# LBruyne/Scalable-Collaborative-zkSNARK

Measured on AMD Instinct MI355X. Metric: G1 scalar-muls/sec (d_msm) + Fr field-ops/sec (d_sumcheck), 2^20 shares, 1/2/4/8 GPU, higher is better.
Workload: dtype u32

## Files before the change

scalable-collaborative-zksnark_amd/csrc/zk_api.cpp:

```cpp
#include <cstdarg>
#include <cstdio>
#include <cstdlib>
#include <cstring>
#include <mutex>
#include <string>
#include <vector>

#include "zk_ctx.hpp"

namespace zk {

struct TuneKey {
    const char* name;
    long Tuning::*field;
};
static const TuneKey kTuneKeys[] = {
    {"sc_pass_wg", &Tuning::sc_pass_wg}, {"sc_local_g", &Tuning::sc_local_g}, {"sc_local_threads", &Tuning::sc_local_threads}, {"sc_ts", &Tuning::sc_ts}, {"sc_xcd", &Tuning::sc_xcd},
    {"sc_kf", &Tuning::sc_kf}, {"sc_plain_flat", &Tuning::sc_plain_flat}, {"sc_kp", &Tuning::sc_kp}, {"sc_k0", &Tuning::sc_k0},
    {"sc_flat_wg", &Tuning::sc_flat_wg}, {"sc_plain_wg", &Tuning::sc_plain_wg}, {"sc_pre", &Tuning::sc_pre},
    {"sc_pinned_out", &Tuning::sc_pinned_out}, {"sc_t1_device", &Tuning::sc_t1_device}, {"sc_handover", &Tuning::sc_handover},
    {"gate_local_e", &Tuning::gate_local_e}, {"gate_pass_wg", &Tuning::gate_pass_wg},
    {"wiring_local_e", &Tuning::wiring_local_e}, {"wiring_pass_wg", &Tuning::wiring_pass_wg},
    {"multi_local_e", &Tuning::multi_local_e}, {"multi_pass_wg", &Tuning::multi_pass_wg},
    {"perm3_local_e", &Tuning::perm3_local_e}, {"gatew_local_e", &Tuning::gatew_local_e},
    {"lookup_local_e", &Tuning::lookup_local_e}, {"lookupsel_local_e", &Tuning::lookupsel_local_e},
    {"msm_table_dc", &Tuning::msm_table_dc}, {"msm_qstep", &Tuning::msm_qstep}, {"msm_tile", &Tuning::msm_tile}, {"msm_pair", &Tuning::msm_pair},
    {"msm_fixq", &Tuning::msm_fixq}, {"msm_quad", &Tuning::msm_quad}, {"msm_stage", &Tuning::msm_stage}, {"msm_split", &Tuning::msm_split},
    {"msm_np", &Tuning::msm_np}, {"msm_fused_min", &Tuning::msm_fused_min}, {"msm_l2_tiled", &Tuning::msm_l2_tiled}, {"msm_tab_spt", &Tuning::msm_tab_spt}, {"msm_idx_ahead", &Tuning::msm_idx_ahead}, {"msm_share_l1", &Tuning::msm_share_l1}, {"srs_table_batched", &Tuning::srs_table_batched}, {"msm_debug", &Tuning::msm_debug}, {"msm_serial", &Tuning::msm_serial}, {"msm_size_classes", &Tuning::msm_size_classes},
    {"g1_map_by_column", &Tuning::g1_map_by_column}, {"msm_share", &Tuning::msm_share}, {"srs_table_rec", &Tuning::srs_table_rec}, {"msm_size_class_min", &Tuning::msm_size_class_min}, {"msm_small_table_widths", &Tuning::msm_small_table_widths},
};
static Tuning g_tuning;
int tune_set(const char* key, long value) {
    if (!key) return ZK_ERR_INVALID;
    for (const TuneKey& k : kTuneKeys)
        if (!std::strcmp(k.name, key)) {
            tuning().*(k.field) = value;
            return ZK_OK;
        }
    return ZK_ERR_INVALID;
}
Tuning& tuning() {
    static std::once_flag once;
    std::call_once(once, [] {
        const char* e = std::getenv("ZKHIP_TUNE");
        if (!e) return;
        std::string s(e);
        size_t pos = 0;
        while (pos < s.size()) {
            size_t end = s.find(',', pos);
            if (end == std::string::npos) end = s.size();
            const std::string kv = s.substr(pos, end - pos);
            const size_t eq = kv.find('=');
            bool ok = false;
            if (eq != std::string::npos) {
                const std::string k = kv.substr(0, eq);
                for (const TuneKey& t : kTuneKeys)
                    if (k == t.name) {
                        g_tuning.*(t.field) = std::atol(kv.c_str() + eq + 1);
                        ok = true;
                    }
// ... 675 lines not shown
```

scalable-collaborative-zksnark_amd/csrc/zk_ctx.hpp:

```cpp
#pragma once
#include <hip/hip_runtime.h>
#include <stdint.h>
#include <mutex>
#include <string>
#include <unordered_map>
#include <vector>

#include "../../include/zkhip.h"
#include "../../include/zkhip_test.h"

struct zk_msm_job;

struct zk_srs {
    void* d_bases = nullptr;
    size_t n = 0;
    bool owned = true;
    bool g2 = false;
    void* d_table = nullptr;
    int table_c = 0;
    size_t table_stride = 0;
    size_t table_rec = 96;
};

struct zk_ctx {
// ... 65 lines not shown
    long sc_pass_wg = 0;
    long sc_local_g = 256;
    long sc_local_threads = 1024;
    long sc_ts = 0;
    long sc_xcd = 1;
    long sc_kf = 4;
    long sc_plain_flat = 1;
    long sc_kp = 2;
    long sc_k0 = 3;
    long sc_flat_wg = 64;
    long sc_plain_wg = 3;
    long sc_pre = 1;
    long sc_pinned_out = 1;
    long sc_handover = 1;
    long sc_t1_device = 0;
    long gate_local_e = 512;
    long gate_pass_wg = 0;
    long wiring_local_e = 512;
    long wiring_pass_wg = 0;
    long multi_local_e = 512;
    long multi_pass_wg = 0;
    long perm3_local_e = 256;
    long gatew_local_e = 256;
    long lookup_local_e = 512;
    long lookupsel_local_e = 512;
    long msm_table_dc = 0;
    long msm_qstep = 2;
    long msm_tile = 0;
    long msm_pair = 0;
    long msm_fixq = 65536;
    long msm_quad = 32768;
    long msm_stage = -1;
    long msm_split = 1;
    long msm_np = 0;
    long msm_fused_min = 0;
    long msm_share_l1 = 1;
    long msm_idx_ahead = 1;
    long msm_tab_spt = 0;
    long msm_l2_tiled = 0;
    long msm_debug = 0;
    long msm_serial = 0;
    long msm_size_classes = 1;
    long srs_table_batched = 1;
    long srs_table_rec = 0;
    long msm_size_class_min = 16;
    long msm_small_table_widths = 1;
    long msm_share = 100;
    long g1_map_by_column = 1;
};
Tuning& tuning();
int tune_set(const char* key, long value);

int fail(zk_ctx* ctx, int code, const char* fmt, ...);
int hip_fail(zk_ctx* ctx, hipError_t e, const char* what);
void* scratch(zk_ctx* ctx, int slot, size_t bytes);
void* pinned(zk_ctx* ctx, size_t bytes);
hipError_t device_alloc(zk_ctx* ctx, void** out, size_t bytes, bool pool_locked = false);
size_t pool_trim(zk_ctx* ctx);
int msm_lanes_reserve(zk_ctx* ctx, int lane, const uint64_t* caps10, uint64_t pinned_cap);

#define ZK_HIP(ctx, call)                                            \
    do {                                                             \
        hipError_t _e = (call);                                      \
        if (_e != hipSuccess) return zk::hip_fail(ctx, _e, #call);   \
    } while (0)

// ... 100 lines not shown
```

scalable-collaborative-zksnark_amd/csrc/zk_msm.hip:

```cpp
#include "curve30.cuh"
#include "curve30_g2.cuh"
#include "host_curve.hpp"
#include "zk_ctx.hpp"

#include <algorithm>
#include <chrono>
#include <cstdio>
#include <cstdlib>
#include <condition_variable>
#include <cstring>
#include <deque>
#include <functional>
#include <mutex>
#include <thread>
#include <vector>

namespace zk {

static constexpr int kBlk = 256;
static constexpr u32 kSkip = 0xffffffffu;


struct CvG1 {
    typedef Aff30 Aff;
// ... 858 lines not shown
    return 0;
}
static void tab_launch_hist(int c, dim3 grid, hipStream_t st, const ItemDesc* items, WinLayout L, u32 chunk_sc, u32 nchunks, u32 np, int low_bits, u32* hist) {
    switch (c) {
#define X(Cc) case Cc: hipLaunchKernelGGL(k_tab_hist<Cc>, grid, dim3(kSortThreads), 0, st, items, L, chunk_sc, nchunks, np, low_bits, hist); break;
        ZK_TAB_WIDTHS(X)
#undef X
        default: hipLaunchKernelGGL(k_tab_hist<0>, grid, dim3(kSortThreads), 0, st, items, L, chunk_sc, nchunks, np, low_bits, hist);
    }
}
template <int SPT, int C>
static void tab_launch_scatter_one(dim3 grid, size_t lds, hipStream_t st, const ItemDesc* items, u32 ns, WinLayout L, u32 nchunks, u32 np, int low_bits, const u32* hist,
                                   const u32* ptotal, const u32* base, int idx_bits, size_t row_len, u32* part_idx, unsigned short* part_low) {
    hipFuncSetAttribute((const void*)k_tab_scatter<SPT, C>, hipFuncAttributeMaxDynamicSharedMemorySize, 160 * 1024);
    hipLaunchKernelGGL((k_tab_scatter<SPT, C>), grid, dim3(kSortThreads), lds, st, items, ns, L, nchunks, np, low_bits, hist, ptotal, base, idx_bits, row_len, part_idx, part_low);
}
static void tab_launch_scatter(int c, int spt, dim3 grid, size_t lds, hipStream_t st, const ItemDesc* items, u32 ns, WinLayout L, u32 nchunks, u32 np, int low_bits,
                               const u32* hist, const u32* ptotal, const u32* base, int idx_bits, size_t row_len, u32* part_idx, unsigned short* part_low) {
#define ZK_ARGS grid, lds, st, items, ns, L, nchunks, np, low_bits, hist, ptotal, base, idx_bits, row_len, part_idx, part_low
    switch (c) {
#define X(Cc) case Cc: if (spt == 2) tab_launch_scatter_one<2, Cc>(ZK_ARGS); else tab_launch_scatter_one<1, Cc>(ZK_ARGS); break;
        ZK_TAB_WIDTHS(X)
#undef X
        default: if (spt == 2) tab_launch_scatter_one<2, 0>(ZK_ARGS); else tab_launch_scatter_one<1, 0>(ZK_ARGS);
    }
#undef ZK_ARGS
}

template <class Cv>
static __global__ void __launch_bounds__(kBlk) k_accum_tiles(const ItemDesc* __restrict__ items, int rows_per_item,
                                                    const u32* __restrict__ sorted, const uint2* __restrict__ oc_all,
                                                    const u32* __restrict__ tile_b, size_t ns, u32 nsi, int nsi_shift, size_t nb, u32 T,
                                                    size_t tiles_per_w, size_t total_tiles, void* __restrict__ buckets,
                                                    void* __restrict__ heads, void* __restrict__ tails, int idx_ahead) {
  for (size_t g = (size_t)blockIdx.x * kBlk + threadIdx.x; g < total_tiles; g += (size_t)gridDim.x * kBlk) {
    const size_t w = g / tiles_per_w, t = g % tiles_per_w;
    const ItemDesc it = items[w / rows_per_item];
    const void* __restrict__ bases = it.bases;
    auto pidx = [&](u32 v) -> size_t {
        v &= 0x7fffffffu;
        if (it.pstride == 0) return v;
        const u32 win = nsi_shift >= 0 ? (v >> nsi_shift) : v / nsi;
        return (size_t)win * it.pstride + (v - win * nsi);
    };
    const uint2* oc = oc_all + w * nb;
    const uint2 last = oc[nb - 1];
    const u32 nw = last.x + last.y;
    const u32 e0 = (u32)t * T;
    if (e0 >= nw) continue;
    const u32 e1 = (e0 + T < nw) ? e0 + T : nw;
    u32 b = tile_b[g];
    uint2 cur_b = oc[b];
    u32 bstart = cur_b.x, bend = cur_b.x + cur_b.y;
    u32 ps = e0;
    const u32* run = sorted + w * ns;
    typename Cv::Xyzz acc;
    Cv::set_inf(acc);
    u32 v = run[e0];
    u32 vn = (idx_ahead && e0 + 1 < e1) ? run[e0 + 1] : 0u;
    typename Cv::Aff p = Cv::aff_load_rec(bases, pidx(v), it.rec);
    for (u32 e = e0; e < e1; e++) {
        if (e == bend) {
            if (ps == bstart) Cv::store(buckets, w * nb + b, acc);
            else Cv::store(heads, g, acc);
            do {
                b++;
                cur_b = oc[b];
                bstart = cur_b.x;
                bend = cur_b.x + cur_b.y;
            } while (bend == bstart);
            ps = e;
            Cv::set_inf(acc);
        }
        const bool neg = (v >> 31) != 0;
        typename Cv::Aff cur = p;
        if (e + 1 < e1) {
            if (idx_ahead) {
                v = vn;
                if (e + 2 < e1) vn = run[e + 2];
            } else {
                v = run[e + 1];
            }
            p = Cv::aff_load_rec(bases, pidx(v), it.rec);
        }
        Cv::madd(acc, cur, neg);
    }
    if (ps == bstart && e1 == bend) Cv::store(buckets, w * nb + b, acc);
    else if (ps == e0) Cv::store(heads, g, acc);
    else Cv::store(tails, g, acc);
  }
}

struct NarrowRows {
    int rpi, w0, from;
    __host__ __device__ bool narrow(size_t row) const { return w0 + (int)(row % (size_t)rpi) >= from; }
};

static constexpr u32 kLongSpan = 24;
template <class Cv>
static __global__ void __launch_bounds__(kBlk) k_fixup(const uint2* __restrict__ oc, size_t nb, NarrowRows nr, u32 T,
                                              size_t tiles_per_w, size_t total, void* __restrict__ buckets,
                                              const void* __restrict__ heads, const void* __restrict__ tails,
                                              u32* __restrict__ long_count, u32* __restrict__ long_list) {
    const size_t g = (size_t)blockIdx.x * kBlk + threadIdx.x;
    if (g >= total) return;
    const size_t w = g / nb;
    if (nr.narrow(w) && (g % nb) >= nb / 2) return;
    const uint2 ocg = oc[g];
    const u32 s = ocg.x, c = ocg.y;
    if (c == 0) {
        typename Cv::Xyzz z;
        Cv::set_inf(z);
        Cv::store(buckets, g, z);
        return;
    }
    const u32 e = s + c;
    const u32 t0 = s / T, t1 = (e - 1) / T;
    if (t0 == t1) return;
    if (t1 - t0 > kLongSpan) {
        long_list[atomicAdd(long_count, 1u)] = (u32)g;
        return;
    }
    const size_t base = w * tiles_per_w;
    typename Cv::Xyzz acc = (s == t0 * T) ? Cv::load(heads, base + t0) : Cv::load(tails, base + t0);
    for (u32 t = t0 + 1; t <= t1; t++) acc = Cv::add(acc, Cv::load(heads, base + t));
    Cv::store(buckets, g, acc);
}

template <class Cv>
static __global__ void __launch_bounds__(kBlk) k_fixup_quad(const uint2* __restrict__ oc, size_t nb, NarrowRows nr, u32 T,
                                                   size_t tiles_per_w, size_t total, void* __restrict__ buckets,
                                                   const void* __restrict__ heads, const void* __restrict__ tails,
                                                   u32* __restrict__ long_count, u32* __restrict__ long_list) {
    const size_t tq = (size_t)blockIdx.x * kBlk + threadIdx.x;
    const size_t g = tq >> 2;
    const int role = (int)(tq & 3);
    if (g >= total) return;
    const size_t w = g / nb;
    if (nr.narrow(w) && (g % nb) >= nb / 2) return;
    const uint2 ocg = oc[g];
    const u32 s = ocg.x, c = ocg.y;
    if (c == 0) {
        Cv::quad_store_inf(buckets, g, role);
        return;
    }
    const u32 e = s + c;
    const u32 t0 = s / T, t1 = (e - 1) / T;
    if (t0 == t1) return;
    if (t1 - t0 > kLongSpan) {
        if (role == 0) long_list[atomicAdd(long_count, 1u)] = (u32)g;
        return;
    }
    const size_t base = w * tiles_per_w;
    typename Cv::Xyzz acc = (s == t0 * T) ? Cv::load(heads, base + t0) : Cv::load(tails, base + t0);
    for (u32 t = t0 + 1; t <= t1; t++) acc = Cv::acc_quad(acc, heads, base + t, role);
    Cv::quad_store(buckets, g, role, acc);
}

template <class Cv>
static __global__ void __launch_bounds__(kBlk) k_fixup_long(const uint2* __restrict__ oc, size_t nb, u32 T,
                                                   size_t tiles_per_w, void* __restrict__ buckets, const void* __restrict__ heads,
                                                   const void* __restrict__ tails, const u32* __restrict__ long_count,
                                                   const u32* __restrict__ long_list) {
    extern __shared__ uint4 red[];
    const u32 nlong = *long_count;
    for (u32 i = blockIdx.x; i < nlong; i += gridDim.x) {
        const size_t g = long_list[i];
        const size_t w = g / nb;
// ... 282 lines not shown
    std::memcpy(Y.data(), p + 6, 48);
    std::memcpy(ZZ.data(), p + 12, 48);
    std::memcpy(ZZZ.data(), p + 18, 48);
    if (zkhost::is_zero(ZZ)) return zkhost::jac_inf();
    return zkhost::xyzz_to_jac(zkhost::mul(X, zkhost::K378()), zkhost::mul(Y, zkhost::K378()), zkhost::mul(ZZ, zkhost::K378()),
                               zkhost::mul(ZZZ, zkhost::K378()));
}

template <class HF>
static void combine_windows(zkhost::JacT<HF>& acc, const uint64_t* h, const WinLayout& L, int w0, int wc, int c, int nout, bool pair) {
    typedef zkhost::JacT<HF> J;
    constexpr size_t fw = zkhost::fe_words<HF>();
    const size_t p_lo = (size_t)L.bit_offset(w0);
    const size_t p_hi = (w0 + wc >= L.W) ? (size_t)L.bit_offset(L.W - 1) + L.width(L.W - 1) + c + 2 : (size_t)L.bit_offset(w0 + wc);
    std::vector<J> pos(p_hi - p_lo, zkhost::jac_inf_t<HF>());
    for (int w = 0; w < wc; w++) {
        for (int j = 0; j < nout; j++) {
            const uint64_t* src = h + ((size_t)w * nout + j) * 3 * fw;
            J pt;
            zkhost::get_fe(pt.x, src);
            zkhost::get_fe(pt.y, src + fw);
            zkhost::get_fe(pt.z, src + 2 * fw);
            if (zkhost::is_zero(pt.z)) continue;
            const size_t p = (size_t)L.bit_offset(w0 + w) + (pair ? 2 * (size_t)j : (j == c - 1 ? 0 : (size_t)j)) - p_lo;
            pos[p] = zkhost::jac_add(pos[p], pt);
        }
    }
    for (size_t p = pos.size(); p-- > 0;) {
        acc = zkhost::jac_dbl(acc);
        if (!zkhost::is_zero(pos[p].z)) acc = zkhost::jac_add(acc, pos[p]);
    }
}

struct HostPool {
    std::vector<std::thread> th;
    std::mutex mu;
    std::condition_variable cv, cv_done;
    std::deque<std::function<void()>> q;
    size_t pending = 0;
    bool stop = false;
    explicit HostPool(unsigned n) {
        for (unsigned i = 0; i < n; i++)
            th.emplace_back([this] {
                for (;;) {
                    std::function<void()> job;
                    {
                        std::unique_lock<std::mutex> lk(mu);
                        cv.wait(lk, [this] { return stop || !q.empty(); });
                        if (q.empty()) return;
                        job = std::move(q.front());
                        q.pop_front();
                    }
                    job();
                    {
                        std::lock_guard<std::mutex> lk(mu);
                        if (--pending == 0) cv_done.notify_all();
                    }
                }
            });
    }
    void submit(std::function<void()> f) {
        {
            std::lock_guard<std::mutex> lk(mu);
            q.push_back(std::move(f));
            pending++;
        }
// ... 19 lines not shown
#ifndef ZK_MSM_TU_G2
void msm_host_pool_destroy(zk_ctx* ctx) {
    delete (HostPool*)ctx->host_pool;
    ctx->host_pool = nullptr;
}

#endif
struct MsmClass {
    bool shared = false;
    int rpi = 0;
    size_t row_len = 0;
    int copies = 2;
    int c = 0;
    int key_c = 0;
    int size_key = 0;
    int narrow_from = 0x7fffffff;
    int w0 = 0, wc = 0;
    int part = 0, nparts = 1;
    int npair = 0;
    bool pair = false;
    WinLayout L{};
    std::vector<size_t> idx;
    size_t ns = 0, nb = 0, rows = 0, total = 0, tiles_per_w = 0, total_tiles = 0, chunk_len = 0, cc_elems = 0;
    u32 T = 32, nchunks = 0, np = 1;
    int low_bits = 0;
    int idx_bits = 0;
    bool staged_scatter = false;
    bool fused_tab = false;
    bool tiled_l2 = false;
    u32 tab_spt = 2;
    int tab_c = 0;
    u32 l2_ub = 0;
    size_t pinned_off = 0;
    size_t off[10] = {0, 0, 0, 0, 0, 0, 0, 0, 0, 0};
};

static int quantised_window(int c) {
    const int step = std::max(1, (int)tuning().msm_qstep);
    return c <= 5 ? 5 : (c > 17 ? 19 : std::min(17, 5 + step * ((c - 5 + step - 1) / step)));
}

struct MsmRun {
    int lane = 0;
    bool own_mem = false;
    size_t count = 0;
    std::vector<MsmItem> items;
    std::vector<MsmClass> classes;
    std::vector<size_t> empty_items;
    void* buf[10] = {};
    char* hpin = nullptr;
    size_t pinned_bytes = 0;
    size_t accum_wg_cap = 0;
};

static void msm_release(zk_ctx* ctx, MsmRun& run) {
    if (!run.own_mem || run.lane <= 0) return;
    ctx->lanes[run.lane].busy = false;
    run.lane = -1;
}

static int msm_lane_prepare(zk_ctx* ctx, int lane) {
    zk_ctx::MsmLane& L = ctx->lanes[lane];
    if (lane == 0) L.main = ctx->stream;
    if (L.ready) return ZK_OK;
    ZK_HIP(ctx, hipStreamCreateWithFlags(&L.main, hipStreamNonBlocking));
    for (auto& s2 : L.aux) ZK_HIP(ctx, hipStreamCreateWithFlags(&s2, hipStreamNonBlocking));
// ... 187 lines not shown
            cl.np = (u32)std::min<size_t>(cl.nb, want);
        }
        cl.low_bits = 0;
        while (((size_t)cl.np << cl.low_bits) < cl.nb) cl.low_bits++;
        {
            int ib = 1;
            while (((size_t)1 << ib) < cl.row_len) ib++;
            cl.idx_bits = (ib + cl.low_bits <= 31) ? ib : 0;
        }
        cl.staged_scatter = stage_env >= 0 ? stage_env != 0 : cl.row_len >= ((size_t)1 << 20);
        if (cl.rows * (size_t)cl.np * (cl.row_len / kStageChunk + 1) > ((size_t)64 << 20)) cl.staged_scatter = false;
        cl.chunk_len = cl.staged_scatter ? kStageChunk : (std::max<size_t>(16384, (cl.row_len + 511) / 512) + 3) & ~(size_t)3;
        cl.nchunks = (u32)((cl.row_len + cl.chunk_len - 1) / cl.chunk_len);
        cl.fused_tab = cl.shared && cl.w0 == 0 && cl.wc == cl.L.W && cl.L.W <= kTabW && cl.np == kMaxParts && cl.row_len >= ((size_t)1 << (tn.msm_fused_min > 0 ? tn.msm_fused_min : 23)) &&
                       tn.msm_fused_min >= 0;
        if (cl.fused_tab) {
            cl.tab_spt = cl.L.W <= 16 ? 2 : 1;
            if (tn.msm_tab_spt == 1) cl.tab_spt = 1;
            cl.tab_c = tab_width_known(cl.key_c);
            if (cl.tab_c) {
                const WinLayout chk = msm_layout(cl.tab_c, kFullBits);
                if (chk.W != cl.L.W || chk.base != cl.L.base || chk.rem != cl.L.rem) cl.tab_c = 0;
            }
            const size_t chunk_sc = (size_t)cl.tab_spt * kSortThreads;
            const size_t nch = (cl.ns + chunk_sc - 1) / chunk_sc;
            if (cl.rows * (size_t)cl.np * nch > ((size_t)64 << 20)) cl.fused_tab = false;
            else cl.nchunks = (u32)nch;
        }
        cl.tiled_l2 = tn.msm_l2_tiled >= 0 && cl.row_len / cl.np >= (size_t)(tn.msm_l2_tiled > 0 ? tn.msm_l2_tiled : 8192) && (tn.msm_l2_tiled > 0 || cl.row_len >= ((size_t)1 << 23));
        cl.l2_ub = (u32)(cl.row_len / kL2Tile + cl.np);
        if (cl.tiled_l2 && cl.rows * (size_t)cl.l2_ub * ((size_t)1 << cl.low_bits) > ((size_t)64 << 20)) cl.tiled_l2 = false;
        cl.cc_elems = cl.rows * (size_t)cl.np * cl.nchunks + 2 * cl.rows * (size_t)cl.np + cl.rows;
        if (cl.tiled_l2) cl.cc_elems += cl.rows * (size_t)(cl.np + 1) + cl.rows * (size_t)cl.l2_ub * ((size_t)1 << cl.low_bits);
        const size_t total64 = (cl.total + 63) & ~(size_t)63, tiles64 = (cl.total_tiles + 63) & ~(size_t)63;
        const size_t want_b[10] = {cl.rows * cl.row_len * 4, cl.rows * cl.row_len * 4, 2 * cl.total * 4 + cl.total_tiles * 4, total64 * Cv::kXyzzBytes, total64 * Cv::kXyzzBytes,
                                   2 * tiles64 * Cv::kXyzzBytes, (cl.total_tiles / kLongSpan + 64 + 1) * 4, nitems * sizeof(ItemDesc),
                                   cl.cc_elems * 4, cl.rows * cl.row_len * 2};
        for (int i = 0; i < 10; i++) {
            const bool shared_scratch = share_l1 && (i == 1 || i == 9);
            cl.off[i] = shared_scratch ? 0 : need[i];
            if (shared_scratch) need[i] = std::max(need[i], (want_b[i] + 255) & ~(size_t)255);
            else need[i] += (want_b[i] + 255) & ~(size_t)255;
        }
        cl.pinned_off = pinned_bytes;
        pinned_bytes += ((cl.rows * (size_t)cl.npair * Cv::kJacBytes + 255) & ~(size_t)255) + ((nitems * sizeof(ItemDesc) + 255) & ~(size_t)255);
    }
    const bool dbg_classes = tn.msm_debug != 0;
    if (dbg_classes)
        for (auto& cl : classes) {
            size_t nmin = ~(size_t)0, nmax2 = 0, tot = 0;
            for (size_t k : cl.idx) nmin = std::min(nmin, items[k].n), nmax2 = std::max(nmax2, items[k].n), tot += items[k].n;
            fprintf(stderr, "zk-class key_c=%d c=%d W=%d items=%zu n=[%zu..%zu] sum=%zu ns=%zu rows=%zu nb=%zu buckets=%zu T=%u tiles=%zu np=%u\n", cl.key_c, cl.c, cl.wc,
                    cl.idx.size(), nmin, nmax2, tot, cl.ns, cl.rows, cl.nb, cl.total, cl.T, cl.total_tiles, cl.np);
        }
    static const int slot[10] = {0, 1, 2, 3, 4, 5, 6, 9, 8, 11};
    void** buf = run.buf;
    run.pinned_bytes = pinned_bytes;
    if (run.own_mem) {
        int pick = -1;
        size_t pick_cap = 0;
        bool pick_fits = false;
        for (int l = 1; l < zk_ctx::kLanes; l++) {
            const zk_ctx::MsmLane& cand = ctx->lanes[l];
            if (cand.busy) continue;
            size_t cap = 0;
            bool fits = cand.pinned_cap >= pinned_bytes;
            for (int i = 0; i < 10; i++) cap += cand.mem[i].cap, fits = fits && cand.mem[i].cap >= need[i];
            const bool better = pick < 0 || (fits && !pick_fits) || (fits == pick_fits && (fits ? cap < pick_cap : cap > pick_cap));
            if (better) pick = l, pick_cap = cap, pick_fits = fits;
        }
        if (pick < 0) return fail(ctx, ZK_ERR_INVALID, "too many asynchronous MSM jobs in flight (at most %d): wait for one first", zk_ctx::kLanes - 1);
        run.lane = pick;
        {
            const int rc = msm_lane_prepare(ctx, run.lane);
            if (rc) return rc;
        }
        zk_ctx::MsmLane& LL = ctx->lanes[run.lane];
        for (int i = 0; i < 10; i++) {
            zk_ctx::Arena& a = LL.mem[i];
            if (a.cap < need[i] || !a.p) {
                if (a.p) hipFree(a.p);
                a.p = nullptr, a.cap = 0;
                const size_t want = std::max<size_t>(need[i], 256);
                const hipError_t e = device_alloc(ctx, &a.p, want);
                if (e != hipSuccess) {
                    a.p = nullptr;
// ... 40 lines not shown
    const bool multi = classes.size() > 1 && !serial_env;
    if (multi) {
        hipEventRecord(L.ev_fork, L.main);
        for (int k = 0; k < zk_ctx::kAux; k++) hipStreamWaitEvent(L.aux[k], L.ev_fork, 0);
    }
#define ZK_HIP_INFLIGHT(ctx, call)                                   \
    do {                                                             \
        hipError_t _e = (call);                                      \
        if (_e != hipSuccess) {                                      \
            hipDeviceSynchronize();                                  \
            msm_release(ctx, run);                                   \
            return zk::hip_fail(ctx, _e, #call);                     \
        }                                                            \
    } while (0)
    size_t cls_i = 0;
    for (auto& cl : classes) {
        const size_t nitems = cl.idx.size(), ns = cl.ns, nb = cl.nb, total = cl.total;
        const bool t_first = timers && (cls_i == 0), t_last = timers && (cls_i + 1 == (size_t)classes[0].nparts);
        hipStream_t st = (!multi || cls_i == 0) ? L.main : L.aux[(cls_i - 1) % zk_ctx::kAux];
        u32* digits = (u32*)((char*)buf[0] + cl.off[0]);
        u32* sorted = digits;
        u32* part_idx = (u32*)((char*)buf[1] + cl.off[1]);
        unsigned short* part_low = (unsigned short*)((char*)buf[9] + cl.off[9]);
        uint2* oc = (uint2*)((char*)buf[2] + cl.off[2]);
        u32* tile_b = (u32*)(oc + total);
        void* bufA = (char*)buf[3] + cl.off[3];
        void* bufB = (char*)buf[4] + cl.off[4];
        void* heads = (char*)buf[5] + cl.off[5];
        void* tails = (char*)heads + ((cl.total_tiles + 63) & ~(size_t)63) * Cv::kXyzzBytes;
        u32* longs = (u32*)((char*)buf[6] + cl.off[6]);
        ItemDesc* d_items = (ItemDesc*)((char*)buf[7] + cl.off[7]);
        u32* cc = (u32*)((char*)buf[8] + cl.off[8]);
        uint64_t* h_pts = (uint64_t*)(hpin + cl.pinned_off);
        ItemDesc* h_items = (ItemDesc*)(hpin + cl.pinned_off + ((cl.rows * (size_t)cl.npair * Cv::kJacBytes + 255) & ~(size_t)255));
        for (size_t j = 0; j < nitems; j++) {
            const MsmItem& it = items[cl.idx[j]];
            h_items[j].scalars = it.d_scalars;
            h_items[j].rec = cl.shared ? (u32)it.srs->table_rec : (u32)Cv::kAffBytes;
            h_items[j].bases = (const char*)(cl.shared ? it.srs->d_table : it.srs->d_bases) + it.offset * (size_t)h_items[j].rec;
            h_items[j].n = (u32)it.n;
            h_items[j].pstride = cl.shared ? (u32)it.srs->table_stride : (Cv::kEndo ? (u32)it.srs->n : 0u);
        }
        if (t_first) hipEventRecord(ctx->ev[0], st);
        ZK_HIP_INFLIGHT(ctx, hipMemcpyAsync(d_items, h_items, nitems * sizeof(ItemDesc), hipMemcpyHostToDevice, st));
        ZK_HIP_INFLIGHT(ctx, hipMemsetAsync(longs, 0, 4, st));
        if (share_l1) {
            while (L.ev_sort.size() <= cls_i) {
                hipEvent_t e = nullptr;
                ZK_HIP_INFLIGHT(ctx, hipEventCreateWithFlags(&e, hipEventDisableTiming));
                L.ev_sort.push_back(e);
            }
            if (cls_i > 0) hipStreamWaitEvent(st, L.ev_sort[cls_i - 1], 0);
        }
        if (!cl.fused_tab)
            hipLaunchKernelGGL(k_digits, dim3((unsigned)((ns + kBlk - 1) / kBlk), (unsigned)nitems), dim3(kBlk), 0, st,
                               (const ItemDesc*)d_items, ns, cl.L, cl.w0, cl.wc, (cl.shared || !Cv::kEndo) ? 0 : 1, digits);
        {
            u32* hist = cc;
            u32* ptotal = hist + cl.rows * (size_t)cl.np * cl.nchunks;
            u32* pbase = ptotal + cl.rows * (size_t)cl.np;
            u32* rowtot = pbase + cl.rows * (size_t)cl.np;
            const dim3 g_chunks((unsigned)(cl.nchunks * cl.rows)), g_parts((unsigned)(cl.np * cl.rows));
            const RowReal rr{(const ItemDesc*)d_items, (u32)cl.rpi, (u32)ns};
            if (cl.fused_tab)
                tab_launch_hist(cl.tab_c, g_chunks, st, (const ItemDesc*)d_items, cl.L, cl.tab_spt * (u32)kSortThreads, cl.nchunks, cl.np, cl.low_bits, hist);
            else
                hipLaunchKernelGGL(k_part_hist, g_chunks, dim3(kSortThreads), 0, st, (const u32*)digits, cl.row_len, cl.chunk_len, cl.nchunks, cl.np,
// ... 5 lines not shown
                tab_launch_scatter(cl.tab_c, (int)cl.tab_spt, dim3((unsigned)(8 * ((cl.nchunks + 7) / 8) * cl.rows)), lds, st, (const ItemDesc*)d_items, (u32)ns, cl.L, cl.nchunks, cl.np, cl.low_bits, (const u32*)hist,
                                   (const u32*)ptotal, (const u32*)pbase, cl.idx_bits, cl.row_len, part_idx, part_low);
            } else if (cl.staged_scatter) {
                const size_t lds = (3 * (size_t)kMaxParts + kSortThreads + 2 * (size_t)kStageChunk) * 4;
                hipFuncSetAttribute((const void*)k_part_scatter_staged, hipFuncAttributeMaxDynamicSharedMemorySize, 160 * 1024);
                hipLaunchKernelGGL(k_part_scatter_staged, g_chunks, dim3(kSortThreads), lds, st, (const u32*)digits, cl.row_len, cl.chunk_len,
                                   cl.nchunks, cl.np, cl.low_bits, (const u32*)hist, (const u32*)pbase, cl.idx_bits, part_idx, part_low, rr);
            } else {
                hipLaunchKernelGGL(k_part_scatter, g_chunks, dim3(kSortThreads), 0, st, (const u32*)digits, cl.row_len, cl.chunk_len, cl.nchunks,
                                   cl.np, cl.low_bits, (const u32*)hist, (const u32*)pbase, cl.idx_bits, part_idx, part_low, rr);
            }
            if (cl.tiled_l2) {
                u32* tstart = rowtot + cl.rows;
                u32* h2 = tstart + cl.rows * (size_t)(cl.np + 1);
                const u32 ub = cl.l2_ub;
                const dim3 g_tiles((unsigned)(ub * cl.rows));
                const size_t lds = (2 * ((size_t)1 << cl.low_bits) + 1 + 160 + kL2Tile) * 4;
                hipLaunchKernelGGL(k_l2_tiles, dim3((unsigned)cl.rows), dim3(kScanThreads), 0, st, (const u32*)pbase, (const u32*)rowtot, cl.np, tstart);
                hipLaunchKernelGGL(k_l2_hist, g_tiles, dim3(kSortThreads), 0, st, (const u32*)part_idx, (const unsigned short*)part_low, cl.row_len, cl.np, cl.low_bits, cl.idx_bits,
                                   (const u32*)pbase, (const u32*)rowtot, (const u32*)tstart, ub, h2);
                hipLaunchKernelGGL(k_l2_scan, g_parts, dim3(kSortThreads), 0, st, cl.np, cl.low_bits, nb, (const u32*)pbase, (const u32*)tstart, ub, h2, oc, cl.T, cl.tiles_per_w, tile_b);
                hipFuncSetAttribute((const void*)k_l2_scatter, hipFuncAttributeMaxDynamicSharedMemorySize, 160 * 1024);
                hipLaunchKernelGGL(k_l2_scatter, dim3((unsigned)(8 * ((ub + 7) / 8) * cl.rows)), dim3(kSortThreads), lds, st, (const u32*)part_idx, (const unsigned short*)part_low, cl.row_len, cl.np, cl.low_bits,
                                   cl.idx_bits, nb, (const u32*)pbase, (const u32*)rowtot, (const u32*)tstart, ub, (const u32*)h2, (const uint2*)oc, sorted);
            } else
            hipLaunchKernelGGL(k_part_sort, g_parts, dim3(cl.row_len / cl.np >= 4096 ? kSortThreads : 256), 0, st, (const u32*)part_idx, (const unsigned short*)part_low, cl.row_len,
                               cl.np, cl.low_bits, cl.idx_bits, nb, (const u32*)pbase, (const u32*)rowtot, oc, cl.T, cl.tiles_per_w, tile_b, sorted);
        }
        if (share_l1) hipEventRecord(L.ev_sort[cls_i], st);
        if (t_first) hipEventRecord(ctx->ev[1], st);
        if (cl.part > 0) hipStreamWaitEvent(st, L.ev_part[(cl.part - 1) % zk_ctx::kParts], 0);
        const size_t accum_wgs_full = (cl.total_tiles + kBlk - 1) / kBlk;
        const size_t accum_wgs = run.accum_wg_cap ? std::min<size_t>(accum_wgs_full, run.accum_wg_cap) : accum_wgs_full;
        hipLaunchKernelGGL((k_accum_tiles<Cv>), dim3((unsigned)accum_wgs), dim3(kBlk), 0, st,
                           (const ItemDesc*)d_items, cl.rpi, (const u32*)sorted, (const uint2*)oc, (const u32*)tile_b, cl.row_len,
                           (u32)ns, ((ns & (ns - 1)) == 0) ? (int)__builtin_ctzll(ns) : -1, nb, cl.T, cl.tiles_per_w, cl.total_tiles, bufA, heads, tails, (int)tn.msm_idx_ahead);
        if (cl.nparts > 1 && cl.part + 1 < cl.nparts) hipEventRecord(L.ev_part[cl.part % zk_ctx::kParts], st);
        if (t_last) hipEventRecord(ctx->ev[4], st);
        const NarrowRows nrw{cl.rpi, cl.w0, cl.narrow_from};
        if (Cv::kQuad && total <= fixq_max)
            hipLaunchKernelGGL((k_fixup_quad<Cv>), dim3((unsigned)((4 * total + kBlk - 1) / kBlk)), dim3(kBlk), 0, st, (const uint2*)oc,
                               nb, nrw, cl.T, cl.tiles_per_w, total, bufA, (const void*)heads, (const void*)tails, longs,
                               longs + 1);
        else
            hipLaunchKernelGGL((k_fixup<Cv>), dim3((unsigned)((total + kBlk - 1) / kBlk)), dim3(kBlk), 0, st, (const uint2*)oc,
                               nb, nrw, cl.T, cl.tiles_per_w, total, bufA, (const void*)heads, (const void*)tails, longs,
                               longs + 1);
        hipLaunchKernelGGL((k_fixup_long<Cv>), dim3(512), dim3(Cv::kXyzzBytes == 192 ? kBlk : kBlk / 2), (size_t)48 * 1024, st, (const uint2*)oc, nb, cl.T,
                           cl.tiles_per_w, bufA, (const void*)heads, (const void*)tails, (const u32*)longs, (const u32*)(longs + 1));
        if (t_last) hipEventRecord(ctx->ev[2], st);
        void* in = bufA;
        void* out = bufB;
        int rows = 1;
        size_t len = nb;
        while (len > 1) {
            size_t threads = cl.rows * (size_t)(rows + 1) * (len >> 1);
            if (Cv::kQuad && threads <= quad_max)
                hipLaunchKernelGGL((k_halve_quad<Cv>), dim3((unsigned)((4 * threads + kBlk - 1) / kBlk)), dim3(kBlk), 0, st, (const void*)in, out,
                                   (int)cl.rows, rows, len, nrw);
            else
                hipLaunchKernelGGL((k_halve<Cv>), dim3((unsigned)((threads + kBlk - 1) / kBlk)), dim3(kBlk), 0, st, (const void*)in, out,
                                   (int)cl.rows, rows, len, nrw);
            std::swap(in, out);
            rows++;
            len >>= 1;
        }
        {
            const size_t threads = cl.rows * (size_t)cl.npair;
            hipLaunchKernelGGL((k_finish<Cv>), dim3((unsigned)((threads + 63) / 64)), dim3(64), 0, st, (const void*)in, out, cl.rows, cl.c, cl.npair, cl.pair ? 1 : 0);
        }
        ZK_HIP_INFLIGHT(ctx, hipGetLastError());
        ZK_HIP_INFLIGHT(ctx, hipMemcpyAsync(h_pts, out, cl.rows * (size_t)cl.npair * Cv::kJacBytes, hipMemcpyDeviceToHost, st));
        if (t_last) hipEventRecord(ctx->ev[3], st);
        while (L.ev_cls.size() <= cls_i) {
            hipEvent_t e;
            ZK_HIP_INFLIGHT(ctx, hipEventCreateWithFlags(&e, hipEventDisableTiming));
            L.ev_cls.push_back(e);
        }
        hipEventRecord(L.ev_cls[cls_i], st);
        cls_i++;
    }
#undef ZK_HIP_INFLIGHT
    if (multi) {
        for (int k = 0; k < zk_ctx::kAux; k++) {
            hipEventRecord(L.ev_join[k], L.aux[k]);
            hipStreamWaitEvent(L.main, L.ev_join[k], 0);
        }
    }
    return ZK_OK;
}

template <class Cv>
static int msm_finish(zk_ctx* ctx, MsmRun& run, uint64_t* h_out) {
    typedef typename Cv::HostF HF;
    constexpr size_t kOutWords = 3 * zkhost::fe_words<HF>();
    const size_t count = run.count;
    std::vector<MsmClass>& classes = run.classes;
    zk_ctx::MsmLane& L = ctx->lanes[run.lane];
    char* hpin = run.hpin;
    for (size_t k : run.empty_items) zkhost::write_normalised(zkhost::jac_inf_t<HF>(), h_out + kOutWords * k);
    if (classes.empty()) return ZK_OK;
    std::vector<zkhost::JacT<HF>> chain(count, zkhost::jac_inf_t<HF>());
    auto run_item = [&chain, hpin, h_out](const MsmClass& cl, size_t j) {
        WinLayout one{1, 0, 0};
        const uint64_t* h = (const uint64_t*)(hpin + cl.pinned_off) + j * (size_t)cl.rpi * cl.npair * kOutWords;
        if (cl.shared) combine_windows<HF>(chain[cl.idx[j]], h, one, 0, 1, cl.c, cl.npair, cl.pair);
        else combine_windows<HF>(chain[cl.idx[j]], h, cl.L, cl.w0, cl.wc, cl.c, cl.npair, cl.pair);
        if (cl.part + 1 == cl.nparts) zkhost::write_normalised(chain[cl.idx[j]], h_out + kOutWords * cl.idx[j]);
    };
    std::vector<size_t> order(classes.size());
    for (size_t i = 0; i < order.size(); i++) order[i] = i;
    std::stable_sort(order.begin(), order.end(), [&](size_t a, size_t b) {
        const MsmClass &x = classes[a], &y = classes[b];
        if (x.nparts > 1 || y.nparts > 1) return a < b;
        return x.rows * x.row_len < y.rows * y.row_len;
    });
    HostPool* pool = classes.size() > 1 || count > 1 ? host_pool(ctx) : nullptr;
    float host_ms = 0;
    for (size_t oi = 0; oi < order.size(); oi++) {
        const MsmClass& cl = classes[order[oi]];
        {
            const hipError_t e = hipEventSynchronize(L.ev_cls[order[oi]]);
            if (e != hipSuccess) {
                if (pool) pool->wait();
                msm_release(ctx, run);
                return hip_fail(ctx, e, "hipEventSynchronize(class done)");
            }
        }
        auto t0 = std::chrono::steady_clock::now();
        if (cl.nparts > 1 && cl.part > 0 && pool) pool->wait();
        for (size_t j = 0; j < cl.idx.size(); j++) {
            if (pool && (cl.idx.size() > 1 || oi + 1 < order.size())) pool->submit([&run_item, &cl, j] { run_item(cl, j); });
            else run_item(cl, j);
        }
        if (oi + 1 == order.size()) {
            if (pool) pool->wait();
            host_ms = std::chrono::duration<float, std::milli>(std::chrono::steady_clock::now() - t0).count();
        }
    }
    {
        const hipError_t e = hipStreamSynchronize(L.main);
        msm_release(ctx, run);
        if (e != hipSuccess) return hip_fail(ctx, e, "hipStreamSynchronize(msm lane)");
    }
    if (run.lane != 0) return ZK_OK;
    float ms;
    hipEventElapsedTime(&ms, ctx->ev[0], ctx->ev[1]);
    ctx->msm_ms[0] = ms;
    hipEventElapsedTime(&ms, ctx->ev[1], ctx->ev[4]);
    ctx->msm_ms[1] = ms;
    hipEventElapsedTime(&ms, ctx->ev[4], ctx->ev[2]);
    ctx->msm_ms[2] = ms;
    hipEventElapsedTime(&ms, ctx->ev[2], ctx->ev[3]);
    ctx->msm_ms[3] = ms;
    ctx->msm_ms[4] = host_ms;
    ctx->msm_ms[5] = ctx->msm_ms[0] + ctx->msm_ms[1] + ctx->msm_ms[2] + ctx->msm_ms[3] + ctx->msm_ms[4];
    return ZK_OK;
}

template <class Cv>
static int msm_batch(zk_ctx* ctx, const MsmItem* items, size_t count, uint64_t* h_out) {
    if (!h_out && count) return fail(ctx, ZK_ERR_INVALID, "null argument");
    MsmRun run;
// ... 418 lines not shown
```

Before: 396.1 million.

## Split MSM bucket range into parts to overlap accumulation, reduction and host fold

For a single large shared MSM class, the bucket space is split into several ranges. Accumulation kernels now run per tile range, and each range's fixup and halving reduction runs on an auxiliary stream, so later accumulation overlaps earlier tails. Each range's partial bucket sums are copied back separately and folded on the host with binary position weights while the GPU keeps working. This adds kernel launches, events and host-side curve arithmetic, and the per-range reductions carry extra correctness risk.

```diff
diff --git a/scalable-collaborative-zksnark_amd/csrc/zk_api.cpp b/scalable-collaborative-zksnark_amd/csrc/zk_api.cpp
--- a/scalable-collaborative-zksnark_amd/csrc/zk_api.cpp
+++ b/scalable-collaborative-zksnark_amd/csrc/zk_api.cpp
@@ -25,7 +25,7 @@
     {"perm3_local_e", &Tuning::perm3_local_e}, {"gatew_local_e", &Tuning::gatew_local_e},
     {"lookup_local_e", &Tuning::lookup_local_e}, {"lookupsel_local_e", &Tuning::lookupsel_local_e},
     {"msm_table_dc", &Tuning::msm_table_dc}, {"msm_qstep", &Tuning::msm_qstep}, {"msm_tile", &Tuning::msm_tile}, {"msm_pair", &Tuning::msm_pair},
-    {"msm_fixq", &Tuning::msm_fixq}, {"msm_quad", &Tuning::msm_quad}, {"msm_stage", &Tuning::msm_stage}, {"msm_split", &Tuning::msm_split},
+    {"msm_fixq", &Tuning::msm_fixq}, {"msm_quad", &Tuning::msm_quad}, {"msm_stage", &Tuning::msm_stage}, {"msm_split", &Tuning::msm_split}, {"msm_bsplit", &Tuning::msm_bsplit}, {"msm_bsplit_min", &Tuning::msm_bsplit_min}, {"msm_bsplit_shape", &Tuning::msm_bsplit_shape},
     {"msm_np", &Tuning::msm_np}, {"msm_fused_min", &Tuning::msm_fused_min}, {"msm_l2_tiled", &Tuning::msm_l2_tiled}, {"msm_tab_spt", &Tuning::msm_tab_spt}, {"msm_idx_ahead", &Tuning::msm_idx_ahead}, {"msm_share_l1", &Tuning::msm_share_l1}, {"srs_table_batched", &Tuning::srs_table_batched}, {"msm_debug", &Tuning::msm_debug}, {"msm_serial", &Tuning::msm_serial}, {"msm_size_classes", &Tuning::msm_size_classes},
     {"g1_map_by_column", &Tuning::g1_map_by_column}, {"msm_share", &Tuning::msm_share}, {"srs_table_rec", &Tuning::srs_table_rec}, {"msm_size_class_min", &Tuning::msm_size_class_min}, {"msm_small_table_widths", &Tuning::msm_small_table_widths},
 };
diff --git a/scalable-collaborative-zksnark_amd/csrc/zk_ctx.hpp b/scalable-collaborative-zksnark_amd/csrc/zk_ctx.hpp
--- a/scalable-collaborative-zksnark_amd/csrc/zk_ctx.hpp
+++ b/scalable-collaborative-zksnark_amd/csrc/zk_ctx.hpp
@@ -121,6 +121,9 @@
     long msm_quad = 32768;
     long msm_stage = -1;
     long msm_split = 1;
+    long msm_bsplit = 1;
+    long msm_bsplit_min = 17;
+    long msm_bsplit_shape = 2;
     long msm_np = 0;
     long msm_fused_min = 0;
     long msm_share_l1 = 1;
diff --git a/scalable-collaborative-zksnark_amd/csrc/zk_msm.hip b/scalable-collaborative-zksnark_amd/csrc/zk_msm.hip
--- a/scalable-collaborative-zksnark_amd/csrc/zk_msm.hip
+++ b/scalable-collaborative-zksnark_amd/csrc/zk_msm.hip
@@ -914,8 +914,14 @@
                                                     const u32* __restrict__ sorted, const uint2* __restrict__ oc_all,
                                                     const u32* __restrict__ tile_b, size_t ns, u32 nsi, int nsi_shift, size_t nb, u32 T,
                                                     size_t tiles_per_w, size_t total_tiles, void* __restrict__ buckets,
-                                                    void* __restrict__ heads, void* __restrict__ tails, int idx_ahead) {
-  for (size_t g = (size_t)blockIdx.x * kBlk + threadIdx.x; g < total_tiles; g += (size_t)gridDim.x * kBlk) {
+                                                    void* __restrict__ heads, void* __restrict__ tails, int idx_ahead,
+                                                    const u32* __restrict__ tile_range) {
+  size_t g_lo = 0, g_hi = total_tiles;
+  if (tile_range) {
+    g_lo = tile_range[0];
+    g_hi = tile_range[1] < total_tiles ? tile_range[1] : total_tiles;
+  }
+  for (size_t g = g_lo + (size_t)blockIdx.x * kBlk + threadIdx.x; g < g_hi; g += (size_t)gridDim.x * kBlk) {
     const size_t w = g / tiles_per_w, t = g % tiles_per_w;
     const ItemDesc it = items[w / rows_per_item];
     const void* __restrict__ bases = it.bases;
@@ -973,6 +979,31 @@
   }
 }
 
+struct BucketRanges {
+    int n, desc;
+    u32 off[zk_ctx::kParts], len[zk_ctx::kParts];
+};
+static __global__ void __launch_bounds__(64) k_range_tiles(const uint2* __restrict__ oc, size_t nb, u32 T, BucketRanges br, u32* __restrict__ tile_range,
+                                                  u32* __restrict__ longs, size_t long_stride) {
+    const int p = (int)threadIdx.x;
+    if (p >= br.n) return;
+    const uint2 last = oc[nb - 1];
+    const u32 nw = last.x + last.y;
+    const size_t end = (size_t)br.off[p] + br.len[p];
+    const u32 s = oc[br.off[p]].x, e = end < nb ? oc[end].x : nw;
+    u32 lo, hi;
+    if (br.desc) {
+        lo = s / T;
+        hi = end < nb ? e / T : (nw + T - 1) / T;
+    } else {
+        lo = (s + T - 1) / T;
+        hi = (e + T - 1) / T;
+    }
+    tile_range[2 * p] = lo;
+    tile_range[2 * p + 1] = hi;
+    longs[(size_t)p * long_stride] = 0u;
+}
+
 struct NarrowRows {
     int rpi, w0, from;
     __host__ __device__ bool narrow(size_t row) const { return w0 + (int)(row % (size_t)rpi) >= from; }
@@ -981,10 +1012,10 @@
 static constexpr u32 kLongSpan = 24;
 template <class Cv>
 static __global__ void __launch_bounds__(kBlk) k_fixup(const uint2* __restrict__ oc, size_t nb, NarrowRows nr, u32 T,
-                                              size_t tiles_per_w, size_t total, void* __restrict__ buckets,
+                                              size_t tiles_per_w, size_t g0, size_t total, void* __restrict__ buckets,
                                               const void* __restrict__ heads, const void* __restrict__ tails,
                                               u32* __restrict__ long_count, u32* __restrict__ long_list) {
-    const size_t g = (size_t)blockIdx.x * kBlk + threadIdx.x;
+    const size_t g = g0 + (size_t)blockIdx.x * kBlk + threadIdx.x;
     if (g >= total) return;
     const size_t w = g / nb;
     if (nr.narrow(w) && (g % nb) >= nb / 2) return;
@@ -1011,11 +1042,11 @@
 
 template <class Cv>
 static __global__ void __launch_bounds__(kBlk) k_fixup_quad(const uint2* __restrict__ oc, size_t nb, NarrowRows nr, u32 T,
-                                                   size_t tiles_per_w, size_t total, void* __restrict__ buckets,
+                                                   size_t tiles_per_w, size_t g0, size_t total, void* __restrict__ buckets,
                                                    const void* __restrict__ heads, const void* __restrict__ tails,
                                                    u32* __restrict__ long_count, u32* __restrict__ long_list) {
     const size_t tq = (size_t)blockIdx.x * kBlk + threadIdx.x;
-    const size_t g = tq >> 2;
+    const size_t g = g0 + (tq >> 2);
     const int role = (int)(tq & 3);
     if (g >= total) return;
     const size_t w = g / nb;
@@ -1364,6 +1395,34 @@
     }
 }
 
+template <class HF>
+static void fold_bucket_range(std::vector<zkhost::JacT<HF>>& pos, const uint64_t* h, int m, size_t off) {
+    typedef zkhost::JacT<HF> J;
+    constexpr size_t fw = zkhost::fe_words<HF>();
+    for (int j = 0; j <= m; j++) {
+        const uint64_t* src = h + (size_t)j * 3 * fw;
+        J pt;
+        zkhost::get_fe(pt.x, src);
+        zkhost::get_fe(pt.y, src + fw);
+        zkhost::get_fe(pt.z, src + 2 * fw);
+        if (zkhost::is_zero(pt.z)) continue;
+        if (j < m) {
+            pos[j] = zkhost::jac_add(pos[j], pt);
+        } else {
+            const size_t weight = 1 + off;
+            for (size_t k = 0; (weight >> k) != 0; k++)
+                if ((weight >> k) & 1) pos[k] = zkhost::jac_add(pos[k], pt);
+        }
+    }
+}
+template <class HF>
+static void run_positions(zkhost::JacT<HF>& acc, const std::vector<zkhost::JacT<HF>>& pos) {
+    for (size_t p = pos.size(); p-- > 0;) {
+        acc = zkhost::jac_dbl(acc);
+        if (!zkhost::is_zero(pos[p].z)) acc = zkhost::jac_add(acc, pos[p]);
+    }
+}
+
 struct HostPool {
     std::vector<std::thread> th;
     std::mutex mu;
@@ -1449,6 +1508,9 @@
     int tab_c = 0;
     u32 l2_ub = 0;
     size_t pinned_off = 0;
+    size_t pts_bytes = 0;
+    int bparts = 1, bdesc = 0, bm[zk_ctx::kParts] = {};
+    size_t boff[zk_ctx::kParts] = {}, blen[zk_ctx::kParts] = {}, pts_slot = 0, long_stride = 0;
     size_t off[10] = {0, 0, 0, 0, 0, 0, 0, 0, 0, 0};
 };
 
@@ -1702,9 +1764,31 @@
         if (cl.tiled_l2 && cl.rows * (size_t)cl.l2_ub * ((size_t)1 << cl.low_bits) > ((size_t)64 << 20)) cl.tiled_l2 = false;
         cl.cc_elems = cl.rows * (size_t)cl.np * cl.nchunks + 2 * cl.rows * (size_t)cl.np + cl.rows;
         if (cl.tiled_l2) cl.cc_elems += cl.rows * (size_t)(cl.np + 1) + cl.rows * (size_t)cl.l2_ub * ((size_t)1 << cl.low_bits);
+        {
+            int P = std::min((int)tn.msm_bsplit, (int)zk_ctx::kParts);
+            const bool can = classes.size() == 1 && cl.shared && nitems == 1 && !cl.pair && P >= 2 && tn.msm_bsplit_min < 40 && cl.nb >= ((size_t)1 << std::max(0L, tn.msm_bsplit_min));
+            const bool equal = (tn.msm_bsplit_shape & 1) != 0;
+            if (can && equal && P == 3) P = 2;
+            while (can && P >= 2 && (equal ? cl.nb / P : cl.nb >> (P - 1)) < 64) P = equal ? P / 2 : P - 1;
+            if (can && P >= 2) {
+                cl.bparts = P;
+                cl.bdesc = (tn.msm_bsplit_shape & 2) ? 1 : 0;
+                size_t at = 0;
+                for (int p = 0; p < P; p++) {
+                    const size_t len = equal ? cl.nb / P : (p + 1 < P ? cl.nb >> (p + 1) : cl.nb >> (P - 1));
+                    cl.boff[p] = at, cl.blen[p] = len;
+                    at += len;
+                }
+                if (cl.bdesc)
+                    for (int p = 0; p < P; p++) cl.boff[p] = cl.nb - cl.boff[p] - cl.blen[p];
+                for (int p = 0; p < P; p++) cl.bm[p] = (int)__builtin_ctzll(cl.blen[p]);
+                cl.pts_slot = ((size_t)cl.c * Cv::kJacBytes + 255) & ~(size_t)255;
+            }
+            cl.long_stride = cl.total_tiles / kLongSpan + 64 + 1;
+        }
         const size_t total64 = (cl.total + 63) & ~(size_t)63, tiles64 = (cl.total_tiles + 63) & ~(size_t)63;
-        const size_t want_b[10] = {cl.rows * cl.row_len * 4, cl.rows * cl.row_len * 4, 2 * cl.total * 4 + cl.total_tiles * 4, total64 * Cv::kXyzzBytes, total64 * Cv::kXyzzBytes,
-                                   2 * tiles64 * Cv::kXyzzBytes, (cl.total_tiles / kLongSpan + 64 + 1) * 4, nitems * sizeof(ItemDesc),
+        const size_t want_b[10] = {cl.rows * cl.row_len * 4, cl.rows * cl.row_len * 4, 2 * cl.total * 4 + cl.total_tiles * 4 + (cl.bparts > 1 ? 2 * zk_ctx::kParts * 4 : 0), total64 * Cv::kXyzzBytes, total64 * Cv::kXyzzBytes,
+                                   2 * tiles64 * Cv::kXyzzBytes, cl.long_stride * 4 * (size_t)cl.bparts, nitems * sizeof(ItemDesc),
                                    cl.cc_elems * 4, cl.rows * cl.row_len * 2};
         for (int i = 0; i < 10; i++) {
             const bool shared_scratch = share_l1 && (i == 1 || i == 9);
@@ -1713,15 +1797,18 @@
             else need[i] += (want_b[i] + 255) & ~(size_t)255;
         }
         cl.pinned_off = pinned_bytes;
-        pinned_bytes += ((cl.rows * (size_t)cl.npair * Cv::kJacBytes + 255) & ~(size_t)255) + ((nitems * sizeof(ItemDesc) + 255) & ~(size_t)255);
+        cl.pts_bytes = cl.bparts > 1 ? (size_t)cl.bparts * cl.pts_slot : ((cl.rows * (size_t)cl.npair * Cv::kJacBytes + 255) & ~(size_t)255);
+        pinned_bytes += cl.pts_bytes + ((nitems * sizeof(ItemDesc) + 255) & ~(size_t)255);
     }
     const bool dbg_classes = tn.msm_debug != 0;
     if (dbg_classes)
         for (auto& cl : classes) {
             size_t nmin = ~(size_t)0, nmax2 = 0, tot = 0;
             for (size_t k : cl.idx) nmin = std::min(nmin, items[k].n), nmax2 = std::max(nmax2, items[k].n), tot += items[k].n;
-            fprintf(stderr, "zk-class key_c=%d c=%d W=%d items=%zu n=[%zu..%zu] sum=%zu ns=%zu rows=%zu nb=%zu buckets=%zu T=%u tiles=%zu np=%u\n", cl.key_c, cl.c, cl.wc,
-                    cl.idx.size(), nmin, nmax2, tot, cl.ns, cl.rows, cl.nb, cl.total, cl.T, cl.total_tiles, cl.np);
+            fprintf(stderr, "zk-class key_c=%d c=%d W=%d items=%zu n=[%zu..%zu] sum=%zu ns=%zu rows=%zu nb=%zu buckets=%zu T=%u tiles=%zu np=%u branges=%d", cl.key_c, cl.c, cl.wc,
+                    cl.idx.size(), nmin, nmax2, tot, cl.ns, cl.rows, cl.nb, cl.total, cl.T, cl.total_tiles, cl.np, cl.bparts);
+            for (int p = 0; p < cl.bparts && cl.bparts > 1; p++) fprintf(stderr, " [%zu+%zu]", cl.boff[p], cl.blen[p]);
+            fprintf(stderr, "\n");
         }
     static const int slot[10] = {0, 1, 2, 3, 4, 5, 6, 9, 8, 11};
     void** buf = run.buf;
@@ -1828,7 +1915,7 @@
         ItemDesc* d_items = (ItemDesc*)((char*)buf[7] + cl.off[7]);
         u32* cc = (u32*)((char*)buf[8] + cl.off[8]);
         uint64_t* h_pts = (uint64_t*)(hpin + cl.pinned_off);
-        ItemDesc* h_items = (ItemDesc*)(hpin + cl.pinned_off + ((cl.rows * (size_t)cl.npair * Cv::kJacBytes + 255) & ~(size_t)255));
+        ItemDesc* h_items = (ItemDesc*)(hpin + cl.pinned_off + cl.pts_bytes);
         for (size_t j = 0; j < nitems; j++) {
             const MsmItem& it = items[cl.idx[j]];
             h_items[j].scalars = it.d_scalars;
@@ -1900,46 +1987,90 @@
         if (cl.part > 0) hipStreamWaitEvent(st, L.ev_part[(cl.part - 1) % zk_ctx::kParts], 0);
         const size_t accum_wgs_full = (cl.total_tiles + kBlk - 1) / kBlk;
         const size_t accum_wgs = run.accum_wg_cap ? std::min<size_t>(accum_wgs_full, run.accum_wg_cap) : accum_wgs_full;
-        hipLaunchKernelGGL((k_accum_tiles<Cv>), dim3((unsigned)accum_wgs), dim3(kBlk), 0, st,
-                           (const ItemDesc*)d_items, cl.rpi, (const u32*)sorted, (const uint2*)oc, (const u32*)tile_b, cl.row_len,
-                           (u32)ns, ((ns & (ns - 1)) == 0) ? (int)__builtin_ctzll(ns) : -1, nb, cl.T, cl.tiles_per_w, cl.total_tiles, bufA, heads, tails, (int)tn.msm_idx_ahead);
-        if (cl.nparts > 1 && cl.part + 1 < cl.nparts) hipEventRecord(L.ev_part[cl.part % zk_ctx::kParts], st);
-        if (t_last) hipEventRecord(ctx->ev[4], st);
         const NarrowRows nrw{cl.rpi, cl.w0, cl.narrow_from};
-        if (Cv::kQuad && total <= fixq_max)
-            hipLaunchKernelGGL((k_fixup_quad<Cv>), dim3((unsigned)((4 * total + kBlk - 1) / kBlk)), dim3(kBlk), 0, st, (const uint2*)oc,
-                               nb, nrw, cl.T, cl.tiles_per_w, total, bufA, (const void*)heads, (const void*)tails, longs,
-                               longs + 1);
-        else
-            hipLaunchKernelGGL((k_fixup<Cv>), dim3((unsigned)((total + kBlk - 1) / kBlk)), dim3(kBlk), 0, st, (const uint2*)oc,
-                               nb, nrw, cl.T, cl.tiles_per_w, total, bufA, (const void*)heads, (const void*)tails, longs,
-                               longs + 1);
-        hipLaunchKernelGGL((k_fixup_long<Cv>), dim3(512), dim3(Cv::kXyzzBytes == 192 ? kBlk : kBlk / 2), (size_t)48 * 1024, st, (const uint2*)oc, nb, cl.T,
-                           cl.tiles_per_w, bufA, (const void*)heads, (const void*)tails, (const u32*)longs, (const u32*)(longs + 1));
-        if (t_last) hipEventRecord(ctx->ev[2], st);
-        void* in = bufA;
-        void* out = bufB;
-        int rows = 1;
-        size_t len = nb;
-        while (len > 1) {
-            size_t threads = cl.rows * (size_t)(rows + 1) * (len >> 1);
-            if (Cv::kQuad && threads <= quad_max)
-                hipLaunchKernelGGL((k_halve_quad<Cv>), dim3((unsigned)((4 * threads + kBlk - 1) / kBlk)), dim3(kBlk), 0, st, (const void*)in, out,
-                                   (int)cl.rows, rows, len, nrw);
+        auto enqueue_accum = [&](size_t wgs, const u32* range) {
+            hipLaunchKernelGGL((k_accum_tiles<Cv>), dim3((unsigned)wgs), dim3(kBlk), 0, st,
+                               (const ItemDesc*)d_items, cl.rpi, (const u32*)sorted, (const uint2*)oc, (const u32*)tile_b, cl.row_len,
+                               (u32)ns, ((ns & (ns - 1)) == 0) ? (int)__builtin_ctzll(ns) : -1, nb, cl.T, cl.tiles_per_w, cl.total_tiles, bufA, heads, tails, (int)tn.msm_idx_ahead, range);
+        };
+        auto enqueue_tail = [&](hipStream_t ts, size_t g0, size_t gcount, size_t rlen, int cred, int nout, u32* lng, uint64_t* h_dst, bool timed) -> hipError_t {
+            if (Cv::kQuad && gcount <= fixq_max)
+                hipLaunchKernelGGL((k_fixup_quad<Cv>), dim3((unsigned)((4 * gcount + kBlk - 1) / kBlk)), dim3(kBlk), 0, ts, (const uint2*)oc,
+                                   nb, nrw, cl.T, cl.tiles_per_w, g0, g0 + gcount, bufA, (const void*)heads, (const void*)tails, lng,
+                                   lng + 1);
             else
-                hipLaunchKernelGGL((k_halve<Cv>), dim3((unsigned)((threads + kBlk - 1) / kBlk)), dim3(kBlk), 0, st, (const void*)in, out,
-                                   (int)cl.rows, rows, len, nrw);
-            std::swap(in, out);
-            rows++;
-            len >>= 1;
-        }
-        {
-            const size_t threads = cl.rows * (size_t)cl.npair;
-            hipLaunchKernelGGL((k_finish<Cv>), dim3((unsigned)((threads + 63) / 64)), dim3(64), 0, st, (const void*)in, out, cl.rows, cl.c, cl.npair, cl.pair ? 1 : 0);
-        }
-        ZK_HIP_INFLIGHT(ctx, hipGetLastError());
-        ZK_HIP_INFLIGHT(ctx, hipMemcpyAsync(h_pts, out, cl.rows * (size_t)cl.npair * Cv::kJacBytes, hipMemcpyDeviceToHost, st));
-        if (t_last) hipEventRecord(ctx->ev[3], st);
+                hipLaunchKernelGGL((k_fixup<Cv>), dim3((unsigned)((gcount + kBlk - 1) / kBlk)), dim3(kBlk), 0, ts, (const uint2*)oc,
+                                   nb, nrw, cl.T, cl.tiles_per_w, g0, g0 + gcount, bufA, (const void*)heads, (const void*)tails, lng,
+                                   lng + 1);
+            hipLaunchKernelGGL((k_fixup_long<Cv>), dim3(512), dim3(Cv::kXyzzBytes == 192 ? kBlk : kBlk / 2), (size_t)48 * 1024, ts, (const uint2*)oc, nb, cl.T,
+                               cl.tiles_per_w, bufA, (const void*)heads, (const void*)tails, (const u32*)lng, (const u32*)(lng + 1));
+            if (timed) hipEventRecord(ctx->ev[2], ts);
+            void* in = (char*)bufA + g0 * Cv::kXyzzBytes;
+            void* out = (char*)bufB + g0 * Cv::kXyzzBytes;
+            int rows = 1;
+            size_t len = rlen;
+            while (len > 1) {
+                size_t threads = cl.rows * (size_t)(rows + 1) * (len >> 1);
+                if (Cv::kQuad && threads <= quad_max)
+                    hipLaunchKernelGGL((k_halve_quad<Cv>), dim3((unsigned)((4 * threads + kBlk - 1) / kBlk)), dim3(kBlk), 0, ts, (const void*)in, out,
+                                       (int)cl.rows, rows, len, nrw);
+                else
+                    hipLaunchKernelGGL((k_halve<Cv>), dim3((unsigned)((threads + kBlk - 1) / kBlk)), dim3(kBlk), 0, ts, (const void*)in, out,
+                                       (int)cl.rows, rows, len, nrw);
+                std::swap(in, out);
+                rows++;
+                len >>= 1;
+            }
+            {
+                const size_t threads = cl.rows * (size_t)nout;
+                hipLaunchKernelGGL((k_finish<Cv>), dim3((unsigned)((threads + 63) / 64)), dim3(64), 0, ts, (const void*)in, out, cl.rows, cred, nout, cl.pair ? 1 : 0);
+            }
+            hipError_t e = hipGetLastError();
+            if (e == hipSuccess) e = hipMemcpyAsync(h_dst, out, cl.rows * (size_t)nout * Cv::kJacBytes, hipMemcpyDeviceToHost, ts);
+            if (timed) hipEventRecord(ctx->ev[3], ts);
+            return e;
+        };
+        if (cl.bparts > 1) {
+            const int P = cl.bparts;
+            u32* tile_range = tile_b + cl.total_tiles;
+            BucketRanges br{P, cl.bdesc, {}, {}};
+            for (int p = 0; p < P; p++) br.off[p] = (u32)cl.boff[p], br.len[p] = (u32)cl.blen[p];
+            hipLaunchKernelGGL(k_range_tiles, dim3(1), dim3(64), 0, st, (const uint2*)oc, nb, cl.T, br, tile_range, longs, cl.long_stride);
+            for (int p = 0; p < P; p++) {
+                double share = 0;
+                for (int w = 0; w < cl.L.W; w++) {
+                    const double reach = (double)((size_t)1 << (cl.L.width(w) - 1));
+                    share += std::max(0.0, std::min(reach, (double)(cl.boff[p] + cl.blen[p])) - (double)cl.boff[p]) / reach;
+                }
+                share /= (double)cl.L.W;
+                const size_t wgs = std::min(accum_wgs, std::max<size_t>((size_t)(1.1 * share * (double)accum_wgs_full) + 2, std::min<size_t>(accum_wgs, (size_t)ctx->cu_count)));
+                enqueue_accum(wgs, (const u32*)(tile_range + 2 * p));
+                if (p + 1 < P) hipEventRecord(L.ev_part[p], st);
+            }
+            if (t_last) hipEventRecord(ctx->ev[4], st);
+            while (L.ev_cls.size() < (size_t)P) {
+                hipEvent_t e;
+                ZK_HIP_INFLIGHT(ctx, hipEventCreateWithFlags(&e, hipEventDisableTiming));
+                L.ev_cls.push_back(e);
+            }
+            for (int p = 0; p < P; p++) {
+                const bool last = p + 1 == P;
+                hipStream_t ts = (last || serial_env) ? st : L.aux[p];
+                if (ts != st) hipStreamWaitEvent(ts, L.ev_part[p], 0);
+                ZK_HIP_INFLIGHT(ctx, enqueue_tail(ts, cl.boff[p], cl.blen[p], cl.blen[p], cl.bm[p] + 1, cl.bm[p] + 1, longs + (size_t)p * cl.long_stride,
+                                                  (uint64_t*)((char*)h_pts + (size_t)p * cl.pts_slot), last && t_last));
+                if (!last) hipEventRecord(L.ev_cls[1 + p], ts);
+            }
+            for (int p = 0; p + 1 < P && !serial_env; p++) {
+                hipEventRecord(L.ev_join[p], L.aux[p]);
+                hipStreamWaitEvent(st, L.ev_join[p], 0);
+            }
+        } else {
+            enqueue_accum(accum_wgs, nullptr);
+            if (cl.nparts > 1 && cl.part + 1 < cl.nparts) hipEventRecord(L.ev_part[cl.part % zk_ctx::kParts], st);
+            if (t_last) hipEventRecord(ctx->ev[4], st);
+            ZK_HIP_INFLIGHT(ctx, enqueue_tail(st, 0, total, nb, cl.c, cl.npair, longs, h_pts, t_last));
+        }
         while (L.ev_cls.size() <= cls_i) {
             hipEvent_t e;
             ZK_HIP_INFLIGHT(ctx, hipEventCreateWithFlags(&e, hipEventDisableTiming));
@@ -1987,6 +2118,18 @@
     float host_ms = 0;
     for (size_t oi = 0; oi < order.size(); oi++) {
         const MsmClass& cl = classes[order[oi]];
+        std::vector<zkhost::JacT<HF>> bpos;
+        if (cl.bparts > 1) {
+            bpos.assign((size_t)cl.c + 2, zkhost::jac_inf_t<HF>());
+            for (int p = 0; p + 1 < cl.bparts; p++) {
+                const hipError_t e = hipEventSynchronize(L.ev_cls[1 + p]);
+                if (e != hipSuccess) {
+                    msm_release(ctx, run);
+                    return hip_fail(ctx, e, "hipEventSynchronize(bucket range done)");
+                }
+                fold_bucket_range<HF>(bpos, (const uint64_t*)(hpin + cl.pinned_off + (size_t)p * cl.pts_slot), cl.bm[p], cl.boff[p]);
+            }
+        }
         {
             const hipError_t e = hipEventSynchronize(L.ev_cls[order[oi]]);
             if (e != hipSuccess) {
@@ -1997,6 +2140,12 @@
         }
         auto t0 = std::chrono::steady_clock::now();
         if (cl.nparts > 1 && cl.part > 0 && pool) pool->wait();
+        if (cl.bparts > 1) {
+            const int p = cl.bparts - 1;
+            fold_bucket_range<HF>(bpos, (const uint64_t*)(hpin + cl.pinned_off + (size_t)p * cl.pts_slot), cl.bm[p], cl.boff[p]);
+            run_positions<HF>(chain[cl.idx[0]], bpos);
+            zkhost::write_normalised(chain[cl.idx[0]], h_out + kOutWords * cl.idx[0]);
+        } else
         for (size_t j = 0; j < cl.idx.size(); j++) {
             if (pool && (cl.idx.size() > 1 || oi + 1 < order.size())) pool->submit([&run_item, &cl, j] { run_item(cl, j); });
             else run_item(cl, j);
```

Measured after the change: 393.9 million. About the same (-0.6%).
